# tensorflow/recommenders

Hardware: NVIDIA H100
Metric: queries/sec brute-force top-K (1Mx64 candidates) (higher is better)
Workload: dtype f32 (fp16 wgmma screening, fp32 accumulate + exact fp32 re-scoring)

## Files before the change

### recommenders_b200/csrc/common.cuh

```cuda
#pragma once
#include <cuda_runtime.h>
#include <stdint.h>
#include <stdio.h>
#include <stdarg.h>

#include "../../include/tfrs_b200.h"

namespace tfrs {

void set_error(const char* fmt, ...);
void count_launch(int n = 1);

#define TFRS_CHECK_ARG(cond, ...)                          \
  do {                                                     \
    if (!(cond)) {                                         \
      ::tfrs::set_error(__VA_ARGS__);                      \
      return TFRS_ERR_INVALID_ARG;                         \
    }                                                      \
  } while (0)

#define TFRS_CUDA(expr)                                                                          \
  do {                                                                                           \
    cudaError_t e__ = (expr);                                                                    \
    if (e__ != cudaSuccess) {                                                                    \
      ::tfrs::set_error("%s:%d %s -> %s", __FILE__, __LINE__, #expr, cudaGetErrorString(e__));   \
      return TFRS_ERR_CUDA;                                                                      \
    }                                                                                            \
  } while (0)

#define TFRS_LAUNCH_CHECK()                                                                      \
  do {                                                                                           \
    ::tfrs::count_launch();                                                                      \
    cudaError_t e__ = cudaGetLastError();                                                        \
    if (e__ != cudaSuccess) {                                                                    \
      ::tfrs::set_error("%s:%d kernel launch -> %s", __FILE__, __LINE__, cudaGetErrorString(e__)); \
      return TFRS_ERR_CUDA;                                                                      \
    }                                                                                            \
  } while (0)

static inline size_t align_up(size_t x, size_t a) { return (x + a - 1) / a * a; }
static inline int64_t ceil_div(int64_t a, int64_t b) { return (a + b - 1) / b; }

__host__ __device__ __forceinline__ bool better(float sa, long long ia, float sb, long long ib) {
  return (sa > sb) || (sa == sb && ia < ib);
}

__device__ __forceinline__ float finite_abs(float v) {
  const float a = fabsf(v);
  return a < INFINITY ? a : 0.f;
}

int sm_count();

static inline unsigned elementwise_grid(long long n) {
  const long long want = ceil_div(n, 256), cap = (long long)sm_count() * 16;
  return (unsigned)(want < cap ? want : cap);
}

int reduce_parts(const float* partial, long long M, long long N, int parts, float* out, long long ld, cudaStream_t st);
int reduce_loss(const float* v, long long n, long long stride, float* loss, cudaStream_t st);

typedef int (*ThrHook)(void* ctx, float* thr, const float* margin, const float* cut, const int* qexp, const int* exp_corpus,
                       long long Q, cudaStream_t st);
int tc_topk_sharded_local(const float* q, int64_t Q, const float* corpus, const void* index_buf, int64_t N, int d, int k,
                          int64_t index_offset, float* out_scores, int64_t* out_idx, void* ws, size_t ws_bytes, void* stream,
                          ThrHook hook, void* hook_ctx);

struct DeviceOnce {
  unsigned char done_[64] = {};
  int dev_ = 0;
  bool need() { if (cudaGetDevice(&dev_) != cudaSuccess) dev_ = 0; dev_ &= 63; return __atomic_load_n(&done_[dev_], __ATOMIC_ACQUIRE) == 0; }
  void done() { __atomic_store_n(&done_[dev_], (unsigned char)1, __ATOMIC_RELEASE); }
};
#define TFRS_DYN_SMEM(kernel, bytes)                                                                              \
  do {                                                                                                            \
    static ::tfrs::DeviceOnce once__;                                                                             \
    if (once__.need()) {                                                                                          \
      TFRS_CUDA(cudaFuncSetAttribute(kernel, cudaFuncAttributeMaxDynamicSharedMemorySize, (int)(bytes)));         \
                                \
      TFRS_CUDA(cudaFuncSetAttribute(kernel, cudaFuncAttributePreferredSharedMemoryCarveout,                        \
                                     (int)cudaSharedmemCarveoutMaxShared));                                         \
      once__.done();                                                                                              \
    }                                                                                                             \
  } while (0)

}
```

### recommenders_b200/csrc/rowselect.cuh

```cuda
#pragma once
#include "common.cuh"
#include <limits.h>

namespace tfrs {

constexpr int RS_THREADS = 256;

__device__ __forceinline__ void bitonic_sort_desc(float* bs, long long* bi, int P) {
  for (int size = 2; size <= P; size <<= 1) {
    for (int stride = size >> 1; stride > 0; stride >>= 1) {
      for (int t = threadIdx.x; t < (P >> 1); t += blockDim.x) {
        int lo = 2 * t - (t & (stride - 1));
        int hi = lo + stride;
        bool desc = ((lo & size) == 0);
        float sl = bs[lo], sh = bs[hi];
        long long il = bi[lo], ih = bi[hi];
        bool hi_better = better(sh, ih, sl, il);
        bool lo_better = better(sl, il, sh, ih);
        if (desc ? hi_better : lo_better) { bs[lo] = sh; bs[hi] = sl; bi[lo] = ih; bi[hi] = il; }
      }
      __syncthreads();
    }
  }
}

static inline int pow2_ceil(int x) { int p = 1; while (p < x) p <<= 1; return p; }
static inline int rowselect_cap(int k) { int c = pow2_ceil(2 * k); return c < 1024 ? 1024 : c; }
static inline size_t rowselect_smem(int cap, size_t extra) { return (size_t)cap * 12 + extra; }

template <class Provider>
__global__ void __launch_bounds__(RS_THREADS)
row_topk_kernel(Provider prov, int k, int cap, float* __restrict__ out_s, long long* __restrict__ out_i,
                int out_ld) {
  extern __shared__ __align__(16) unsigned char rs_smem[];
  long long* bi = reinterpret_cast<long long*>(rs_smem);
  float* bs = reinterpret_cast<float*>(rs_smem + (size_t)cap * 8);
  void* extra = rs_smem + (size_t)cap * 12;
  __shared__ int cnt_sh;
  __shared__ float thr_s_sh;
  __shared__ long long thr_i_sh;
  __shared__ int full_sh;

  const int row = blockIdx.x;
  const int tid = threadIdx.x;
  if (tid == 0) { cnt_sh = 0; full_sh = 0; thr_s_sh = 0.f; thr_i_sh = 0; }
  prov.begin(row, extra);
  __syncthreads();

  const long long total = prov.count(row);
  const int min_room = cap / 4;
  long long pos = 0;
  while (pos < total) {
    __syncthreads();
    const int cnt0 = cnt_sh;
    const bool full = full_sh != 0;
    const float ts = thr_s_sh;
    const long long ti = thr_i_sh;
    __syncthreads();
    const int slab = (int)min((long long)(cap - cnt0), total - pos);
    for (int t = tid; t < slab; t += RS_THREADS) {
      float s; long long i;
      prov.get(row, pos + t, s, i);
      if (!full || better(s, i, ts, ti)) {
        int p = atomicAdd(&cnt_sh, 1);
        bs[p] = s; bi[p] = i;
      }
    }
    __syncthreads();
    pos += slab;
    const int cnt = cnt_sh;
    if (pos < total && cap - cnt >= min_room) continue;
    int P = 2; while (P < cnt) P <<= 1;
    for (int t = cnt + tid; t < P; t += RS_THREADS) { bs[t] = -INFINITY; bi[t] = LLONG_MAX; }
    __syncthreads();
    if (cnt > 1) bitonic_sort_desc(bs, bi, P);
    if (tid == 0) {
      int keep = cnt < k ? cnt : k;
      cnt_sh = keep;
      if (keep == k) { full_sh = 1; thr_s_sh = bs[k - 1]; thr_i_sh = bi[k - 1]; }
    }
  }
  __syncthreads();
  const int n_out = cnt_sh;
  for (int t = tid; t < n_out; t += RS_THREADS) {
    out_s[(long long)row * out_ld + t] = bs[t];
    out_i[(long long)row * out_ld + t] = bi[t];
  }
}

}
```

### recommenders_b200/csrc/topk_tc.cu

```cuda
#include <cuda_fp16.h>
#include <math.h>
#include <stdlib.h>
#include <type_traits>
#include "rowselect.cuh"
#include "tc_ptx.cuh"

namespace tfrs {
namespace tc {

constexpr int TILE_N = 128;
constexpr int TILE_M = 128;
constexpr int QBLK = 256;
constexpr int KSLAB = 64;
constexpr int SLAB_BYTES = TILE_N * 128;
constexpr int HEADER_BYTES = 1024;
constexpr int THREADS = 512;
constexpr int CONSUMER_WARPS = 16;
constexpr int CAND_CAP = 2048;
constexpr int MAX_SAMPLE_STRIDE = 4;
constexpr int FIN_MAX_PARTS = 2 * 132;
constexpr int MAX_BINS = 1024;
constexpr int FP16_TARGET = 15;
constexpr float E_REL = 0.00108f;
constexpr float E_ACC = 0.00013f;

struct SideStats {
  unsigned int max_norm2_bits;
  unsigned int amax_bits;
  int exp;
  int pad;
};
enum { SAMPLE_STRIDED = 0, SAMPLE_NORM = 1 };
constexpr long long NORM_SAMPLE_MIN_N = 1ll << 19;
constexpr int NORM_SAMPLE_DIV = 8;
constexpr double NORM_SAMPLE_TAIL = 1e-4;
constexpr double NORM_SAMPLE_MIN_PHI = 0.35;
constexpr int NORM_PROBES = 256, NORM_PROBE_K = 100;
constexpr float NORM_PROBE_MIN_MEAN = 0.35f, NORM_PROBE_MIN_EACH = 0.25f;
struct IndexHeader {
  SideStats st;
  int d, d_pad, kb, sample;
  long long n, n_tiles;
  float phi;
  float probe_mean, probe_min;
};
__host__ __device__ inline long long norm_sample_tiles(long long N) {
  return N >= NORM_SAMPLE_MIN_N && N < (1ll << 31) ? N / NORM_SAMPLE_DIV / 128 : 0;
}

__device__ __forceinline__ int rescale_exp(float amax) {
  int x = 0;
  if (!(amax > 0.f) || !(amax < INFINITY)) return 0;
  (void)frexpf(amax, &x);
  return FP16_TARGET - x;
}

// ... 529 lines not shown
    int c = 0;
#pragma unroll
    for (int j = 0; j < KPL; ++j) c += (key[j] >= cand) ? 1 : 0;
    c = __reduce_add_sync(0xffffffffu, c);
    if (c >= k) prefix = cand;
  }
  return prefix;
}
__device__ __forceinline__ unsigned int warp_kth_largest_smem(const unsigned int* keys, int n, int k, int lane, unsigned int prefix, int top_bit) {
  for (int bit = top_bit; bit >= 0; --bit) {
    const unsigned int cand = prefix | (1u << bit);
    int c = 0;
    for (int t = lane; t < n; t += 32) c += (keys[t] >= cand) ? 1 : 0;
    c = __reduce_add_sync(0xffffffffu, c);
    if (c >= k) prefix = cand;
  }
  return prefix;
}

template <int KPL>
__device__ __forceinline__ void thresholds_of_row(const float* __restrict__ binmax, int bins_ld, int n_bins, int k, int k_filter,
                                                  const float* __restrict__ margin, float* __restrict__ thr, float* __restrict__ thr_safe,
                                                  unsigned int* __restrict__ overflow, unsigned int* __restrict__ retry, long long row, int lane) {
  const float* src = binmax + row * bins_ld;
  unsigned int key[KPL];
#pragma unroll
  for (int j = 0; j < KPL; ++j) { const int i = j * 32 + lane; key[j] = i < n_bins ? f2key(__ldg(src + i)) : 0u; }
  const float safe = key2f(warp_kth_largest_regs<KPL>(key, k)) - margin[row];
  const float filter = k_filter < k ? key2f(warp_kth_largest_regs<KPL>(key, k_filter)) - margin[row] : safe;
  if (lane == 0) { thr[row] = filter; thr_safe[row] = safe; overflow[row] = 0; retry[row] = 0; }
}
template <int KPL>
__global__ void __launch_bounds__(256)
tc_threshold_kernel(const float* __restrict__ binmax, int bins_ld, int n_bins, int k, int k_filter, const float* __restrict__ margin,
                    float* __restrict__ thr, float* __restrict__ thr_safe, unsigned int* __restrict__ overflow,
                    unsigned int* __restrict__ retry, long long Q, const IndexHeader* __restrict__ hdr, int n_bins_norm) {
  const int lane = threadIdx.x & 31;
  const long long row = ((long long)blockIdx.x * 256 + threadIdx.x) >> 5;
  if (row >= Q) return;
  if (n_bins_norm > 0 && hdr->sample == SAMPLE_NORM) { n_bins = n_bins_norm; k_filter = k; }
  if (KPL > 16 && n_bins <= 512) thresholds_of_row<16>(binmax, bins_ld, n_bins, k, k_filter, margin, thr, thr_safe, overflow, retry, row, lane);
  else thresholds_of_row<KPL>(binmax, bins_ld, n_bins, k, k_filter, margin, thr, thr_safe, overflow, retry, row, lane);
}

enum { FIN_TOPK = 0, FIN_EXCLUDE = 1, FIN_COUNT = 2 };
constexpr int FW_WARPS = 4;

struct FinParams {
  const float* q; const float* corpus; int d; int k; long long index_offset; long long N; long long Q;
  const unsigned int* count; const float* cand_s; const unsigned int* cand_i; int segs; int cap_part;
  const float* cut; float* thr; const float* thr_safe; unsigned int* overflow;
  unsigned int* retry; int retry_pass;
  int cap_keys, cap_band;
  unsigned int* band_idx; int* band_n;
  int allow_short;
  float* out_s; long long* out_i;
  const long long* identifiers; const long long* exclusions; int n_excl; int k_out;
  const float* pos; const int* qexp; const IndexHeader* hdr; int* out_count;
};

__device__ __forceinline__ float exact_score(const float* __restrict__ qs, const float* __restrict__ c, int d) {
  float acc = 0.f;
  if ((d & 31) == 0) {
    for (int kk = 0; kk < d; kk += 32) {
      float4 cv[8];
#pragma unroll
      for (int u = 0; u < 8; ++u) cv[u] = __ldg(reinterpret_cast<const float4*>(c + kk) + u);
#pragma unroll
      for (int u = 0; u < 8; ++u) {
        acc = fmaf(qs[kk + 4 * u], cv[u].x, acc); acc = fmaf(qs[kk + 4 * u + 1], cv[u].y, acc);
        acc = fmaf(qs[kk + 4 * u + 2], cv[u].z, acc); acc = fmaf(qs[kk + 4 * u + 3], cv[u].w, acc);
      }
    }
  } else if ((d & 3) == 0) {
    for (int kk = 0; kk < d; kk += 4) {
      const float4 cv = __ldg(reinterpret_cast<const float4*>(c + kk));
      acc = fmaf(qs[kk], cv.x, acc); acc = fmaf(qs[kk + 1], cv.y, acc);
      acc = fmaf(qs[kk + 2], cv.z, acc); acc = fmaf(qs[kk + 3], cv.w, acc);
    }
  } else {
    for (int kk = 0; kk < d; ++kk) acc = fmaf(qs[kk], __ldg(c + kk), acc);
  }
  return acc;
}

__device__ __forceinline__ void exact_score2(const float* __restrict__ qs, const float* __restrict__ c0, const float* __restrict__ c1,
                                             int d, float& s0, float& s1) {
  if ((d & 31) == 0) {
    float a0 = 0.f, a1 = 0.f;
    for (int kk = 0; kk < d; kk += 32) {
      float4 u0[8], u1[8];
#pragma unroll
      for (int u = 0; u < 8; ++u) { u0[u] = __ldg(reinterpret_cast<const float4*>(c0 + kk) + u); u1[u] = __ldg(reinterpret_cast<const float4*>(c1 + kk) + u); }
#pragma unroll
      for (int u = 0; u < 8; ++u) {
        const float q0 = qs[kk + 4 * u], q1 = qs[kk + 4 * u + 1], q2 = qs[kk + 4 * u + 2], q3 = qs[kk + 4 * u + 3];
        a0 = fmaf(q0, u0[u].x, a0); a1 = fmaf(q0, u1[u].x, a1);
        a0 = fmaf(q1, u0[u].y, a0); a1 = fmaf(q1, u1[u].y, a1);
        a0 = fmaf(q2, u0[u].z, a0); a1 = fmaf(q2, u1[u].z, a1);
        a0 = fmaf(q3, u0[u].w, a0); a1 = fmaf(q3, u1[u].w, a1);
      }
    }
    s0 = a0; s1 = a1;
  } else {
    s0 = exact_score(qs, c0, d); s1 = exact_score(qs, c1, d);
  }
}

__device__ __forceinline__ void exclude_rerank(const unsigned long long* srt, int kf, unsigned long long* akey, long long row,
                                               const FinParams& p, int lane) {
  for (int t = lane; t < kf; t += 32) {
    const unsigned long long e = srt[t];
    const float s = key2f((unsigned int)(e >> 32));
    const long long gi = (long long)rank_key_index(e) + p.index_offset;
    const long long ident = p.identifiers ? __ldg(p.identifiers + gi) : gi;
    bool isin = false;
    for (int x = 0; x < p.n_excl; ++x) isin |= (__ldg(p.exclusions + row * p.n_excl + x) == ident);
    const float adj = (isin ? s - 1.0e5f : s) + 0.0f;
    akey[t] = ((unsigned long long)f2key(adj) << 32) | (unsigned long long)(0xFFFFFFFFu - (unsigned int)t);
  }
  __syncwarp();
  for (int t = lane; t < kf; t += 32) {
    const unsigned long long mine = akey[t];
    int rank = 0;
    for (int j = 0; j < kf; ++j) rank += (akey[j] > mine) ? 1 : 0;
    if (rank < p.k_out) {
      const unsigned long long e = srt[t];
      p.out_s[row * p.k_out + rank] = rank_key_score(e);
      p.out_i[row * p.k_out + rank] = (long long)rank_key_index(e) + p.index_offset;
    }
  }
}

__host__ __device__ inline size_t sel_warp_bytes(int cap_keys, int segs) {
  return (size_t)cap_keys * 4 + (size_t)cap_keys * 2 + (size_t)((segs + 1 + 3) & ~3) * 4;
}
constexpr int SEL_WARPS = 8;

__device__ __forceinline__ bool load_record(const FinParams& p, long long row, const int* soff, int rec, int total_rec,
                                            unsigned int& ix0, float (&sc)[8]) {
  if (rec >= total_rec) return false;
  int lo = 0, hi = p.segs;
  while (hi - lo > 1) { const int mid = (lo + hi) >> 1; if (soff[mid] <= rec) lo = mid; else hi = mid; }
  const long long at = (row * p.segs + lo) * p.cap_part + (rec - soff[lo]);
  ix0 = __ldg(p.cand_i + at);
  const float4 s0 = __ldg(reinterpret_cast<const float4*>(p.cand_s + at * 8));
  const float4 s1 = __ldg(reinterpret_cast<const float4*>(p.cand_s + at * 8) + 1);
  sc[0] = s0.x; sc[1] = s0.y; sc[2] = s0.z; sc[3] = s0.w; sc[4] = s1.x; sc[5] = s1.y; sc[6] = s1.z; sc[7] = s1.w;
  return true;
}

template <int MODE>
__global__ void __launch_bounds__(SEL_WARPS * 32)
tc_select_kernel(const FinParams p) {
  extern __shared__ __align__(16) unsigned char fsm[];
  const int warp = threadIdx.x >> 5, lane = threadIdx.x & 31;
  const long long row = (long long)blockIdx.x * SEL_WARPS + warp;
  if (row >= p.Q || (p.retry_pass && p.retry[row] == 0u)) return;
  unsigned char* base = fsm + (size_t)warp * sel_warp_bytes(p.cap_keys, p.segs);
  unsigned int* keys = reinterpret_cast<unsigned int*>(base);
  unsigned short* loc = reinterpret_cast<unsigned short*>(keys + p.cap_keys);
  int* soff = reinterpret_cast<int*>(loc + p.cap_keys);
  const unsigned int n32 = (unsigned int)p.N;
  unsigned int* band = p.band_idx + row * p.cap_band;

  int carry = 0; bool bad = false;
  for (int s0 = 0; s0 < p.segs; s0 += 32) {
    const int s = s0 + lane;
    int c = 0;
    if (s < p.segs) {
      const unsigned int cc = __ldg(p.count + row * p.segs + s);
      if (cc > (unsigned int)p.cap_part) bad = true; else c = (int)cc;
    }
    const int inc = warp_incl_scan(c, lane);
    if (s < p.segs) soff[s + 1] = carry + inc;
    carry += __shfl_sync(0xffffffffu, inc, 31);
  }
  if (lane == 0) soff[0] = 0;
  if (__any_sync(0xffffffffu, bad)) {
    if (lane == 0) { p.overflow[row] = 1; p.band_n[row] = 0; }
    return;
  }
  __syncwarp();
  const int total_rec = soff[p.segs];
  const float thr_row = p.thr[row];
  if (MODE != FIN_COUNT && total_rec >= 8192) {
    if (lane == 0) { p.overflow[row] = 1; p.band_n[row] = 0; }
    return;
  }

  if (MODE == FIN_COUNT) {
    const float eps = 0.5f * p.cut[row];
    const float pos_s = ldexpf(p.pos[row], p.hdr->st.exp + p.qexp[row]);
    const float hi = pos_s + eps, lo_b = pos_s - eps;
    int definite = 0, m = 0;
    for (int rb = 0; rb < total_rec; rb += 32) {
      unsigned int ix0 = 0, amb = 0; int cnt = 0; float sc[8];
      if (load_record(p, row, soff, rb + lane, total_rec, ix0, sc)) {
#pragma unroll
        for (int j = 0; j < 8; ++j) {
          const bool real = ix0 + j < n32;
          definite += (real && sc[j] > hi) ? 1 : 0;
          const bool a = real && sc[j] > lo_b && !(sc[j] > hi);
          amb |= a ? (1u << j) : 0u; cnt += a ? 1 : 0;
        }
      }
      const int incl = warp_incl_scan(cnt, lane);
      const int tot = __shfl_sync(0xffffffffu, incl, 31);
      if (m + tot <= p.cap_band) {
        int at_pos = m + incl - cnt;
#pragma unroll
        for (int j = 0; j < 8; ++j)
          if (amb & (1u << j)) { band[at_pos] = ix0 + j; ++at_pos; }
      }
      m += tot;
    }
    definite = __reduce_add_sync(0xffffffffu, definite);
    if (lane == 0) {
      if (definite >= p.k) { p.out_count[row] = p.k; p.band_n[row] = 0; p.overflow[row] = 0; }
      else if (m > p.cap_band) { p.overflow[row] = 1; p.band_n[row] = 0; }
      else { p.out_count[row] = definite; p.band_n[row] = m; p.overflow[row] = 0; }
    }
    return;
  }

  int n = 0;
  unsigned int kmax = 0u, kmin = 0xFFFFFFFFu;
  for (int rb = 0; rb < total_rec; rb += 32) {
    float sc[8]; unsigned int ix0 = 0, keep = 0; int cnt = 0;
    if (load_record(p, row, soff, rb + lane, total_rec, ix0, sc)) {
#pragma unroll
      for (int j = 0; j < 8; ++j) {
        const bool kp = sc[j] >= thr_row && ix0 + j < n32;
        keep |= kp ? (1u << j) : 0u; cnt += kp ? 1 : 0;
      }
    }
    const int incl = warp_incl_scan(cnt, lane);
    const int tot = __shfl_sync(0xffffffffu, incl, 31);
    if (n + tot <= p.cap_keys) {
      int at_pos = n + incl - cnt;
#pragma unroll
      for (int j = 0; j < 8; ++j) {
        if (keep & (1u << j)) {
          const unsigned int key = f2key(sc[j] + 0.0f);
          kmax = max(kmax, key); kmin = min(kmin, key);
          keys[at_pos] = key;
          loc[at_pos] = (unsigned short)(((rb + lane) << 3) | j);
          ++at_pos;
        }
      }
    }
    n += tot;
  }
  auto miss = [&]() {
    if (lane == 0) {
      const float safe = p.thr_safe[row];
      if (thr_row > safe) { p.retry[row] = 1; p.thr[row] = safe; } else p.overflow[row] = 1;
      p.band_n[row] = 0;
    }
  };
  if (n > p.cap_keys) { if (lane == 0) { p.overflow[row] = 1; p.band_n[row] = 0; } return; }
  if (n < p.k && !p.allow_short) { miss(); return; }
  __syncwarp();
  if (n < p.k) {
    const bool fits = n <= p.cap_band;
    for (int t = lane; t < n && fits; t += 32) {
      const unsigned int l = loc[t];
      const int rec = (int)(l >> 3);
      int lo = 0, hi = p.segs;
      while (hi - lo > 1) { const int mid = (lo + hi) >> 1; if (soff[mid] <= rec) lo = mid; else hi = mid; }
      band[t] = __ldg(p.cand_i + (row * p.segs + lo) * p.cap_part + (rec - soff[lo])) + (l & 7u);
    }
    if (lane == 0) { p.overflow[row] = fits ? 0u : 1u; p.band_n[row] = fits ? n : 0; }
    return;
  }
  kmax = __reduce_max_sync(0xffffffffu, kmax); kmin = __reduce_min_sync(0xffffffffu, kmin);
  unsigned int tau_key;
  {
    const unsigned int diff = kmax ^ kmin;
    const int top = diff ? (31 - __clz(diff)) : -1;
    const unsigned int prefix0 = top >= 31 ? 0u : (top < 0 ? kmax : (kmax & ~((2u << top) - 1u)));
    if (n <= 512) {
      unsigned int kr[16];
#pragma unroll
      for (int j = 0; j < 16; ++j) { const int t = j * 32 + lane; kr[j] = t < n ? keys[t] : 0u; }
      tau_key = warp_kth_largest_regs<16>(kr, p.k, prefix0, top);
    } else if (n <= 1024) {
      unsigned int kr[32];
#pragma unroll
      for (int j = 0; j < 32; ++j) { const int t = j * 32 + lane; kr[j] = t < n ? keys[t] : 0u; }
      tau_key = warp_kth_largest_regs<32>(kr, p.k, prefix0, top);
    } else {
      tau_key = warp_kth_largest_smem(keys, n, p.k, lane, prefix0, top);
    }
  }
  const float lim = key2f(tau_key) - p.cut[row];
  if (!p.allow_short && (!(lim >= thr_row) || !(lim > -INFINITY))) { miss(); return; }
  const unsigned int lim_key = f2key(lim + 0.0f);
  const unsigned int lt_mask = (1u << lane) - 1u;
  int m = 0;
  for (int tb = 0; tb < n; tb += 32) {
    const int t = tb + lane;
    const bool kp = t < n && keys[t] >= lim_key;
    const unsigned int vote = __ballot_sync(0xffffffffu, kp);
    if (kp) {
      const int at_pos = m + __popc(vote & lt_mask);
      if (at_pos < p.cap_band) {
        const unsigned int l = loc[t];
        const int rec = (int)(l >> 3);
        int lo = 0, hi = p.segs;
        while (hi - lo > 1) { const int mid = (lo + hi) >> 1; if (soff[mid] <= rec) lo = mid; else hi = mid; }
        band[at_pos] = __ldg(p.cand_i + (row * p.segs + lo) * p.cap_part + (rec - soff[lo])) + (l & 7u);
      }
    }
    m += __popc(vote);
  }
  if (lane == 0) {
    if (m > p.cap_band) { p.overflow[row] = 1; p.band_n[row] = 0; }
    else { p.overflow[row] = 0; p.band_n[row] = m; }
  }
}

constexpr int RS_BLOCK = 128;
template <int MODE>
__global__ void __launch_bounds__(RS_BLOCK)
tc_rescore_kernel(const FinParams p) {
  extern __shared__ __align__(16) unsigned char rsm[];
  unsigned long long* sk = reinterpret_cast<unsigned long long*>(rsm);
  float* qs = reinterpret_cast<float*>(sk + p.cap_band);
  unsigned long long* srt = reinterpret_cast<unsigned long long*>(qs + ((p.d + 3) & ~3));
  __shared__ int greater_sh;
  const long long row = blockIdx.x;
  const int tid = threadIdx.x;
  if (p.overflow[row] != 0) return;
  const int m = p.band_n[row];
  if (MODE == FIN_COUNT && m == 0) return;
  for (int t = tid; t < p.d; t += RS_BLOCK) qs[t] = p.q[row * p.d + t];
  if (tid == 0) greater_sh = 0;
  __syncthreads();
  const unsigned int* band = p.band_idx + row * p.cap_band;
  if (MODE == FIN_COUNT) {
    const float pos = p.pos[row];
    int g = 0;
    for (int t = tid; t < m; t += RS_BLOCK) g += (exact_score(qs, p.corpus + (long long)band[t] * p.d, p.d) > pos) ? 1 : 0;
    g = __reduce_add_sync(0xffffffffu, g);
    if ((tid & 31) == 0 && g) atomicAdd(&greater_sh, g);
    __syncthreads();
    if (tid == 0) { const int c = p.out_count[row] + greater_sh; p.out_count[row] = c < p.k ? c : p.k; }
    return;
  }
  if (p.d == 64) {
    constexpr int RPB = RS_BLOCK / 8;
    constexpr int MAXR = 8;
    const int sub = tid & 7, grp = tid >> 3;
    for (int t0 = 0; t0 < m; t0 += RPB * MAXR) {
      float4 a[MAXR], b[MAXR];
#pragma unroll
      for (int r = 0; r < MAXR; ++r) {
        const int t = t0 + r * RPB + grp;
        if (t < m) {
          const float4* src = reinterpret_cast<const float4*>(p.corpus + (long long)band[t] * 64) + sub * 2;
          a[r] = __ldg(src); b[r] = __ldg(src + 1);
        }
      }
      const float q0 = qs[sub * 8], q1 = qs[sub * 8 + 1], q2 = qs[sub * 8 + 2], q3 = qs[sub * 8 + 3];
      const float q4 = qs[sub * 8 + 4], q5 = qs[sub * 8 + 5], q6 = qs[sub * 8 + 6], q7 = qs[sub * 8 + 7];
#pragma unroll
      for (int r = 0; r < MAXR; ++r) {
        const int t = t0 + r * RPB + grp;
        const bool live = t < m;
        float acc = 0.f;
#pragma unroll
        for (int step = 0; step < 8; ++step) {
          if (sub == step && live) {
            acc = fmaf(q0, a[r].x, acc); acc = fmaf(q1, a[r].y, acc); acc = fmaf(q2, a[r].z, acc); acc = fmaf(q3, a[r].w, acc);
            acc = fmaf(q4, b[r].x, acc); acc = fmaf(q5, b[r].y, acc); acc = fmaf(q6, b[r].z, acc); acc = fmaf(q7, b[r].w, acc);
          }
          acc = __shfl_sync(0xffffffffu, acc, (threadIdx.x & 24) | step);
        }
        if (live && sub == 0) sk[t] = rank_key(acc, band[t]);
      }
    }
  } else {
    for (int t = tid; t < m; t += RS_BLOCK) {
      const unsigned int idx = band[t];
      sk[t] = rank_key(exact_score(qs, p.corpus + (long long)idx * p.d, p.d), idx);
    }
  }
  __syncthreads();
  if (MODE == FIN_TOPK && m < p.k)
    for (int t = m + tid; t < p.k; t += RS_BLOCK) { p.out_s[row * p.k + t] = -INFINITY; p.out_i[row * p.k + t] = LLONG_MAX; }
  for (int t = tid; t < m; t += RS_BLOCK) {
    const unsigned long long mine = sk[t];
    int rank = 0;
#pragma unroll 4
    for (int j = 0; j < m; ++j) rank += (sk[j] > mine) ? 1 : 0;
    if (rank < p.k) {
      if (MODE == FIN_TOPK) {
        p.out_s[row * p.k + rank] = rank_key_score(mine);
        p.out_i[row * p.k + rank] = (long long)rank_key_index(mine) + p.index_offset;
      } else {
        srt[rank] = mine;
      }
    }
  }
  if (MODE == FIN_EXCLUDE) {
    __syncthreads();
    if (tid < 32) exclude_rerank(srt, p.k, srt + p.k, row, p, tid);
  }
}

__global__ void __launch_bounds__(FW_WARPS * 32)
tc_exclude_fallback_kernel(const FinParams p, const float* __restrict__ tmp_s, const long long* __restrict__ tmp_i,
                           const unsigned int* __restrict__ was_fallback) {
  extern __shared__ __align__(16) unsigned char fsm[];
  const int warp = threadIdx.x >> 5, lane = threadIdx.x & 31;
  const long long row = (long long)blockIdx.x * FW_WARPS + warp;
  if (row >= p.Q || was_fallback[row] == 0) return;
  unsigned long long* srt = reinterpret_cast<unsigned long long*>(fsm) + (size_t)warp * 2 * p.k;
  unsigned long long* akey = srt + p.k;
  for (int t = lane; t < p.k; t += 32)
    srt[t] = rank_key(tmp_s[row * p.k + t], (unsigned int)(tmp_i[row * p.k + t] - p.index_offset));
  __syncwarp();
  exclude_rerank(srt, p.k, akey, row, p, lane);
}

struct FallbackProvider {
  const float* q; const float* corpus; long long N; int d; long long index_offset; const unsigned int* overflow;
  float* qs;
  __device__ void begin(int row, void* extra) {
    qs = reinterpret_cast<float*>(extra);
    if (overflow[row] != 0) for (int t = threadIdx.x; t < d; t += blockDim.x) qs[t] = q[(long long)row * d + t];
  }
  __device__ long long count(int row) const { return overflow[row] != 0 ? N : 0; }
  __device__ void get(int, long long t, float& s, long long& i) const {
    const float* c = corpus + t * d;
    float acc = 0.f;
    for (int kk = 0; kk < d; ++kk) acc = fmaf(qs[kk], __ldg(c + kk), acc);
    s = acc; i = index_offset + t;
  }
};

__global__ void __launch_bounds__(256)
tc_count_fallback_kernel(const float* __restrict__ q, const float* __restrict__ corpus, long long N, int d, int k,
                         const float* __restrict__ pos, const unsigned int* __restrict__ overflow, int* __restrict__ out_count) {
  __shared__ float qs[128];
  __shared__ int total;
  const int row = blockIdx.x;
  if (overflow[row] == 0) return;
  for (int t = threadIdx.x; t < d; t += 256) qs[t] = q[(long long)row * d + t];
  if (threadIdx.x == 0) total = 0;
  __syncthreads();
  const float ps = pos[row];
  int c = 0;
  for (long long t = threadIdx.x; t < N; t += 256) {
    const float* cr = corpus + t * d;
    float acc = 0.f;
    for (int kk = 0; kk < d; ++kk) acc = fmaf(qs[kk], __ldg(cr + kk), acc);
    c += (acc + 0.0f > ps) ? 1 : 0;
  }
  c = __reduce_add_sync(0xffffffffu, c);
// ... 88 lines not shown
  }
  {
    const double lambda = (double)k * pl.stride / (pl.parts_full * 2.0);
    const double want = 2.0 * lambda + 12.0 * sqrt(lambda) + 8.0;
    int p2 = 32; while (p2 < want && p2 < 512) p2 <<= 1;
    pl.cap_part = p2;
    int ck = 1024; while (ck < 1.6 * 1.3 * k * pl.stride && ck < 4096) ck <<= 1;
    pl.cap_keys = ck;
    pl.cap_band = ck / 2;
  }
  pl.smem = (size_t)(2 + pl.stages) * pl.kb * SLAB_BYTES + 1024  + 256 ;
  size_t o = 0;
  auto take = [&](size_t bytes) { size_t r = o; o += align_up(bytes, 1024); return r; };
  pl.o_qimg = take((size_t)pl.nqb * 2 * pl.kb * SLAB_BYTES);
  pl.o_margin = take((size_t)pl.Qp * 4);
  pl.o_cut = take((size_t)pl.Qp * 4);
  pl.o_thr = take((size_t)pl.Qp * 4);
  pl.o_qexp = take((size_t)pl.Qp * 4);
  pl.o_count = take((size_t)pl.Qp * pl.parts_full * 2 * 4);
  pl.o_ovf = take((size_t)pl.Qp * 4);
  pl.o_binmax = take((size_t)pl.Qp * pl.bins_ld * 4);
  pl.o_cand = take((size_t)pl.Qp * pl.parts_full * 2 * pl.cap_part * (8 * 4 + 4));
  pl.o_tmp = take((size_t)Q * k * 12);
  pl.o_band = take((size_t)pl.Qp * pl.cap_band * 4);
  pl.o_bandn = take((size_t)pl.Qp * 4);
  pl.o_thr_safe = take((size_t)pl.Qp * 4);
  pl.o_retry = take((size_t)pl.Qp * 4);
  pl.total = o;
  return true;
}

template <int KB, int STAGES>
static int launch_scans(const Plan& pl, ScanParams sp, cudaStream_t st, int mode) {
  auto ks = tc_scan_kernel<KB, STAGES, MODE_SAMPLE>;
  auto kf = tc_scan_kernel<KB, STAGES, MODE_FILTER>;
  TFRS_DYN_SMEM(ks, (int)pl.smem);
  TFRS_DYN_SMEM(kf, (int)pl.smem);
  if (mode == MODE_SAMPLE) {
    sp.parts = pl.parts_sample; sp.n_seq = pl.n_sample; sp.stride = pl.stride;
    ks<<<(unsigned)(pl.nqb * sp.parts), THREADS, pl.smem, st>>>(sp);
  } else {
    sp.parts = pl.parts_full; sp.n_seq = (int)pl.n_tiles; sp.stride = 1;
    kf<<<(unsigned)(pl.nqb * sp.parts), THREADS, pl.smem, st>>>(sp);
  }
  TFRS_LAUNCH_CHECK();
  return TFRS_OK;
}

static int launch_scan_mode(const Plan& pl, const ScanParams& sp, cudaStream_t st, int mode) {
  if (pl.kb == 1) return launch_scans<1, 6>(pl, sp, st, mode);
  return launch_scans<2, 4>(pl, sp, st, mode);
}

template <int MODE>
static int launch_finalize(FinParams fp, const Plan& pl, ScanParams sp, bool retry, cudaStream_t st) {
  auto ksel = tc_select_kernel<MODE>;
  auto krs = tc_rescore_kernel<MODE>;
  TFRS_DYN_SMEM(ksel, (int)(SEL_WARPS * sel_warp_bytes(4096, FIN_MAX_PARTS)));
  ksel<<<(unsigned)ceil_div(fp.Q, SEL_WARPS), SEL_WARPS * 32, SEL_WARPS * sel_warp_bytes(fp.cap_keys, fp.segs), st>>>(fp);
  TFRS_LAUNCH_CHECK();
  if (retry) {
    sp.retry = fp.retry;
    const int rc = launch_scan_mode(pl, sp, st, MODE_FILTER);
    if (rc) return rc;
    fp.retry_pass = 1;
    ksel<<<(unsigned)ceil_div(fp.Q, SEL_WARPS), SEL_WARPS * 32, SEL_WARPS * sel_warp_bytes(fp.cap_keys, fp.segs), st>>>(fp);
    TFRS_LAUNCH_CHECK();
  }
  const size_t rs_smem = (size_t)fp.cap_band * 8 + (size_t)((fp.d + 3) & ~3) * 4 + (MODE == FIN_EXCLUDE ? (size_t)fp.k * 16 : 0);
  TFRS_DYN_SMEM(krs, 64 * 1024);
  krs<<<(unsigned)fp.Q, RS_BLOCK, rs_smem, st>>>(fp);
  TFRS_LAUNCH_CHECK();
  return TFRS_OK;
}

struct Call {
  int mode;
  const float* q; long long Q; const float* corpus; const void* index_buf; long long N; int d; int k; long long index_offset;
  void* ws; size_t ws_bytes; cudaStream_t st;
  float* out_s; long long* out_i;
  const long long* identifiers; const long long* exclusions; int n_excl; int k_out;
  const float* pos; int* out_count;
  ThrHook hook; void* hook_ctx; int allow_short;
};

static int run_call(const Call& c) {
  Plan pl;
  if (!make_plan(c.Q, c.N, c.d, c.k, pl)) {
    set_error("topk_tc: shape (Q=%lld N=%lld d=%d k=%d) is outside the tensor-core path; use tfrs_topk_scan_f32",
              c.Q, c.N, c.d, c.k);
    return TFRS_ERR_UNSUPPORTED;
  }
  if (!c.ws || c.ws_bytes < pl.total + 16) { set_error("topk_tc: workspace too small (%zu < %zu)", c.ws_bytes, pl.total + 16); return TFRS_ERR_WORKSPACE_TOO_SMALL; }
  TFRS_CHECK_ARG((c.d & 3) != 0 || (reinterpret_cast<uintptr_t>(c.corpus) & 15) == 0,
                 "topk_tc: the corpus must be 16-byte aligned when d %% 4 == 0 (d=%d); pass an aligned copy", c.d);
  cudaStream_t st = c.st;
  unsigned char* w = (unsigned char*)(((uintptr_t)c.ws + 15) & ~(uintptr_t)15);
  unsigned char* qimg = w + pl.o_qimg;
  float* margin = (float*)(w + pl.o_margin);
  float* cut = (float*)(w + pl.o_cut);
  float* thr = (float*)(w + pl.o_thr);
  int* qexp = (int*)(w + pl.o_qexp);
  unsigned int* count = (unsigned int*)(w + pl.o_count);
  unsigned int* ovf = (unsigned int*)(w + pl.o_ovf);
  float* binmax = (float*)(w + pl.o_binmax);
  float* cand_s = (float*)(w + pl.o_cand);
  unsigned int* cand_i = (unsigned int*)(w + pl.o_cand + (size_t)pl.Qp * pl.parts_full * 2 * pl.cap_part * 32);
  float* tmp_s = (float*)(w + pl.o_tmp);
  long long* tmp_i = (long long*)(w + pl.o_tmp + align_up((size_t)c.Q * c.k * 4, 8));
  float* thr_safe = (float*)(w + pl.o_thr_safe);
  unsigned int* retry = (unsigned int*)(w + pl.o_retry);
  const IndexHeader* hdr = (const IndexHeader*)c.index_buf;
  const unsigned char* cimg = (const unsigned char*)c.index_buf + HEADER_BYTES;
  const int k_filter = (c.mode == FIN_COUNT || c.hook) ? c.k : pl.k_filter;

  prof_mark(st, 0);
  tc_qprep_kernel<<<(unsigned)ceil_div(pl.Qp * 32, 256), 256, 0, st>>>(c.q, c.Q, pl.Qp, c.d, pl.kb, hdr, qimg, margin, cut, qexp);
  TFRS_LAUNCH_CHECK();
  ScanParams sp{};
  sp.qimg = qimg; sp.cimg = cimg; sp.Q = c.Q; sp.N = c.N; sp.nqb = pl.nqb; sp.n_tiles = pl.n_tiles;
  sp.binmax = binmax; sp.bins_ld = pl.bins_ld; sp.group = pl.group; sp.bins_per_part = pl.bins_per_part;
  sp.hdr = hdr;
  sp.simg = pl.n_bins_norm > 0 ? cimg + pl.n_tiles * pl.kb * (long long)SLAB_BYTES : nullptr;
  sp.n_seq_norm = pl.n_seq_norm; sp.group_norm = pl.group_norm; sp.bins_per_part_norm = pl.bins_per_part_norm;
  sp.thr = thr; sp.count = count; sp.cand_s = cand_s; sp.cand_i = cand_i; sp.cap_part = pl.cap_part;
  prof_mark(st, 1);
  int rc = launch_scan_mode(pl, sp, st, MODE_SAMPLE);
  if (rc) return rc;
  if (pl.n_bins <= 512 && pl.n_bins_norm <= 512)
    tc_threshold_kernel<16><<<(unsigned)ceil_div(c.Q * 32, 256), 256, 0, st>>>(binmax, pl.bins_ld, pl.n_bins, c.k, k_filter, margin,
                                                                                 thr, thr_safe, ovf, retry, c.Q, hdr, pl.n_bins_norm);
  else
    tc_threshold_kernel<32><<<(unsigned)ceil_div(c.Q * 32, 256), 256, 0, st>>>(binmax, pl.bins_ld, pl.n_bins, c.k, k_filter, margin,
                                                                                 thr, thr_safe, ovf, retry, c.Q, hdr, pl.n_bins_norm);
  TFRS_LAUNCH_CHECK();
  if (c.hook) {
    rc = c.hook(c.hook_ctx, thr, margin, cut, qexp, &hdr->st.exp, c.Q, st);
    if (rc) return rc;
  }
  prof_mark(st, 2);
  rc = launch_scan_mode(pl, sp, st, MODE_FILTER);
  if (rc) return rc;
  prof_mark(st, 3);
  if (FILTER_ABLATION != FILTER_FULL) { prof_mark(st, 4); return TFRS_OK; }
  FinParams fp{};
  fp.q = c.q; fp.corpus = c.corpus; fp.d = c.d; fp.k = c.k; fp.index_offset = c.index_offset; fp.N = c.N; fp.Q = c.Q;
  fp.count = count; fp.cand_s = cand_s; fp.cand_i = cand_i; fp.segs = pl.parts_full * 2; fp.cap_part = pl.cap_part;
  fp.cut = cut; fp.thr = thr; fp.thr_safe = thr_safe; fp.overflow = ovf; fp.retry = retry; fp.out_s = c.out_s; fp.out_i = c.out_i;
  fp.cap_keys = pl.cap_keys; fp.cap_band = pl.cap_band; fp.allow_short = c.allow_short;
  fp.band_idx = (unsigned int*)(w + pl.o_band); fp.band_n = (int*)(w + pl.o_bandn);
  fp.identifiers = c.identifiers; fp.exclusions = c.exclusions; fp.n_excl = c.n_excl; fp.k_out = c.k_out;
  fp.pos = c.pos; fp.qexp = qexp; fp.hdr = hdr; fp.out_count = c.out_count;
  const bool may_retry = k_filter < c.k;
  if (c.mode == FIN_TOPK) rc = launch_finalize<FIN_TOPK>(fp, pl, sp, may_retry, st);
  else if (c.mode == FIN_EXCLUDE) rc = launch_finalize<FIN_EXCLUDE>(fp, pl, sp, may_retry, st);
  else rc = launch_finalize<FIN_COUNT>(fp, pl, sp, false, st);
  if (rc) return rc;
  if (c.mode == FIN_COUNT) {
    tc_count_fallback_kernel<<<(unsigned)c.Q, 256, 0, st>>>(c.q, c.corpus, c.N, c.d, c.k, c.pos, ovf, c.out_count);
    TFRS_LAUNCH_CHECK();
  } else {
    FallbackProvider prov{c.q, c.corpus, c.N, c.d, c.index_offset, ovf, nullptr};
    int cap = rowselect_cap(c.k);
    TFRS_DYN_SMEM(row_topk_kernel<FallbackProvider>, 64 * 1024);
    float* fs = c.mode == FIN_TOPK ? c.out_s : tmp_s;
    long long* fi = c.mode == FIN_TOPK ? c.out_i : tmp_i;
    row_topk_kernel<FallbackProvider><<<(unsigned)c.Q, RS_THREADS, rowselect_smem(cap, (size_t)c.d * 4), st>>>(prov, c.k, cap, fs, fi, c.k);
    TFRS_LAUNCH_CHECK();
    if (c.mode == FIN_EXCLUDE) {
      tc_exclude_fallback_kernel<<<(unsigned)ceil_div(c.Q, FW_WARPS), FW_WARPS * 32, (size_t)FW_WARPS * 2 * c.k * 8, st>>>(fp, tmp_s, tmp_i, ovf);
      TFRS_LAUNCH_CHECK();
    }
  }
  prof_mark(st, 4);
  return TFRS_OK;
}

}
}

using namespace tfrs;
using namespace tfrs::tc;

extern "C" size_t tfrs_index_bytes(int64_t N, int d) {
  if (N <= 0 || d <= 0 || d > 128) return 0;
  int kb = (d + KSLAB - 1) / KSLAB;
  return (size_t)HEADER_BYTES + (size_t)(ceil_div(N, TILE_N) + norm_sample_tiles(N)) * kb * SLAB_BYTES;
}

extern "C" int tfrs_index_build(const float* corpus, int64_t N, int d, void* index_buf, size_t index_bytes, void* stream) {
  TFRS_CHECK_ARG(corpus && index_buf && N > 0 && d > 0, "index_build: bad arguments");
  if (d > 128) { set_error("index_build: d=%d > 128 is not supported by the tensor-core path", d); return TFRS_ERR_UNSUPPORTED; }
  TFRS_CHECK_ARG(index_bytes >= tfrs_index_bytes(N, d), "index_build: buffer too small");
  TFRS_CHECK_ARG((reinterpret_cast<uintptr_t>(index_buf) & 15) == 0, "index_build: buffer must be 16-byte aligned");
  cudaStream_t st = (cudaStream_t)stream;
  IndexHeader h{};
  h.d = d; h.kb = (d + KSLAB - 1) / KSLAB; h.d_pad = h.kb * KSLAB; h.n = N; h.n_tiles = ceil_div(N, TILE_N);
  TFRS_CUDA(cudaMemsetAsync(index_buf, 0, HEADER_BYTES, st));
  header_kernel<<<1, 1, 0, st>>>(reinterpret_cast<IndexHeader*>(index_buf), h);
  TFRS_LAUNCH_CHECK();
  SideStats* cst = &reinterpret_cast<IndexHeader*>(index_buf)->st;
  const unsigned sgrid = (unsigned)(sm_count() * 8);
  corpus_stats_kernel<0><<<sgrid, 256, 0, st>>>(corpus, N, d, cst);
  TFRS_LAUNCH_CHECK();
  side_exp_kernel<<<1, 1, 0, st>>>(cst);
  TFRS_LAUNCH_CHECK();
  const long long s_tiles = norm_sample_tiles(N);
  if (s_tiles == 0) {
    corpus_stats_kernel<1><<<sgrid, 256, 0, st>>>(corpus, N, d, cst);
    TFRS_LAUNCH_CHECK();
  }
  auto image = [&](long long rows, long long tiles, unsigned char* dst, const int* rowmap) {
    const long long chunks = tiles * TILE_N * (long long)h.kb * 8;
    const unsigned blocks = (unsigned)(ceil_div(chunks, 256) < (1 << 20) ? ceil_div(chunks, 256) : (1 << 20));
    tile_image_kernel<<<blocks, 256, 0, st>>>(corpus, rows, d, h.kb, tiles, cst, dst, rowmap);
  };
  unsigned char* img = (unsigned char*)index_buf + HEADER_BYTES;
  image(N, h.n_tiles, img, nullptr);
  TFRS_LAUNCH_CHECK();
  if (s_tiles == 0) return TFRS_OK;
// ... 175 lines not shown
```

Measured before the change: 3.274 million.

## Add PDL launches, prefetch select loads, and team-based multi-row rescore kernel

Adds programmatic dependent launch (griddepcontrol) to the select, rescore and fallback row-topk kernels so each kernel's prologue can overlap the tail of the previous one. Software-prefetches the next record in the select kernel's band and filter loops, and batches four ballot rounds in band compaction. Restructures the rescore kernel so a block of four warps serves one to four query rows depending on Q, with named barriers, shuffle-distributed band indices and multi-key ranking. This aims to cut launch gaps and latency stalls in the finalize stage, at the cost of more register pressure and more complex barrier logic.

```diff
diff --git a/recommenders_b200/csrc/common.cuh b/recommenders_b200/csrc/common.cuh
--- a/recommenders_b200/csrc/common.cuh
+++ b/recommenders_b200/csrc/common.cuh
@@ -40,6 +40,17 @@
 
 static inline size_t align_up(size_t x, size_t a) { return (x + a - 1) / a * a; }
 static inline int64_t ceil_div(int64_t a, int64_t b) { return (a + b - 1) / b; }
+
+__device__ __forceinline__ void grid_dependency_wait() {
+#if defined(__CUDA_ARCH__) && __CUDA_ARCH__ >= 900
+  asm volatile("griddepcontrol.wait;" ::: "memory");
+#endif
+}
+__device__ __forceinline__ void grid_dependents_launch() {
+#if defined(__CUDA_ARCH__) && __CUDA_ARCH__ >= 900
+  asm volatile("griddepcontrol.launch_dependents;" :::);
+#endif
+}
 
 __host__ __device__ __forceinline__ bool better(float sa, long long ia, float sb, long long ib) {
   return (sa > sb) || (sa == sb && ia < ib);
diff --git a/recommenders_b200/csrc/rowselect.cuh b/recommenders_b200/csrc/rowselect.cuh
--- a/recommenders_b200/csrc/rowselect.cuh
+++ b/recommenders_b200/csrc/rowselect.cuh
@@ -43,6 +43,7 @@
 
   const int row = blockIdx.x;
   const int tid = threadIdx.x;
+  grid_dependency_wait();
   if (tid == 0) { cnt_sh = 0; full_sh = 0; thr_s_sh = 0.f; thr_i_sh = 0; }
   prov.begin(row, extra);
   __syncthreads();
diff --git a/recommenders_b200/csrc/topk_tc.cu b/recommenders_b200/csrc/topk_tc.cu
--- a/recommenders_b200/csrc/topk_tc.cu
+++ b/recommenders_b200/csrc/topk_tc.cu
@@ -2,6 +2,7 @@
 #include <math.h>
 #include <stdlib.h>
 #include <type_traits>
+#include <utility>
 #include "rowselect.cuh"
 #include "tc_ptx.cuh"
 
@@ -637,6 +638,7 @@
   const float* cut; float* thr; const float* thr_safe; unsigned int* overflow;
   unsigned int* retry; int retry_pass;
   int cap_keys, cap_band;
+  int rs_team;
   unsigned int* band_idx; int* band_n;
   int allow_short;
   float* out_s; long long* out_i;
@@ -739,6 +741,8 @@
 __global__ void __launch_bounds__(SEL_WARPS * 32)
 tc_select_kernel(const FinParams p) {
   extern __shared__ __align__(16) unsigned char fsm[];
+  grid_dependency_wait();
+  grid_dependents_launch();
   const int warp = threadIdx.x >> 5, lane = threadIdx.x & 31;
   const long long row = (long long)blockIdx.x * SEL_WARPS + warp;
   if (row >= p.Q || (p.retry_pass && p.retry[row] == 0u)) return;
@@ -779,9 +783,12 @@
     const float pos_s = ldexpf(p.pos[row], p.hdr->st.exp + p.qexp[row]);
     const float hi = pos_s + eps, lo_b = pos_s - eps;
     int definite = 0, m = 0;
+    unsigned int ix0 = 0; float sc[8];
+    bool have = load_record(p, row, soff, lane, total_rec, ix0, sc);
     for (int rb = 0; rb < total_rec; rb += 32) {
-      unsigned int ix0 = 0, amb = 0; int cnt = 0; float sc[8];
-      if (load_record(p, row, soff, rb + lane, total_rec, ix0, sc)) {
+      unsigned int nix0 = 0, amb = 0; int cnt = 0; float nsc[8];
+      const bool nhave = load_record(p, row, soff, rb + 32 + lane, total_rec, nix0, nsc);
+      if (have) {
 #pragma unroll
         for (int j = 0; j < 8; ++j) {
           const bool real = ix0 + j < n32;
@@ -799,6 +806,9 @@
           if (amb & (1u << j)) { band[at_pos] = ix0 + j; ++at_pos; }
       }
       m += tot;
+      have = nhave; ix0 = nix0;
+#pragma unroll
+      for (int j = 0; j < 8; ++j) sc[j] = nsc[j];
     }
     definite = __reduce_add_sync(0xffffffffu, definite);
     if (lane == 0) {
@@ -811,9 +821,12 @@
 
   int n = 0;
   unsigned int kmax = 0u, kmin = 0xFFFFFFFFu;
+  float sc[8]; unsigned int ix0 = 0;
+  bool have = load_record(p, row, soff, lane, total_rec, ix0, sc);
   for (int rb = 0; rb < total_rec; rb += 32) {
-    float sc[8]; unsigned int ix0 = 0, keep = 0; int cnt = 0;
-    if (load_record(p, row, soff, rb + lane, total_rec, ix0, sc)) {
+    float nsc[8]; unsigned int nix0 = 0, keep = 0; int cnt = 0;
+    const bool nhave = load_record(p, row, soff, rb + 32 + lane, total_rec, nix0, nsc);
+    if (have) {
 #pragma unroll
       for (int j = 0; j < 8; ++j) {
         const bool kp = sc[j] >= thr_row && ix0 + j < n32;
@@ -836,6 +849,9 @@
       }
     }
     n += tot;
+    have = nhave; ix0 = nix0;
+#pragma unroll
+    for (int j = 0; j < 8; ++j) sc[j] = nsc[j];
   }
   auto miss = [&]() {
     if (lane == 0) {
@@ -884,21 +900,26 @@
   const unsigned int lim_key = f2key(lim + 0.0f);
   const unsigned int lt_mask = (1u << lane) - 1u;
   int m = 0;
-  for (int tb = 0; tb < n; tb += 32) {
-    const int t = tb + lane;
-    const bool kp = t < n && keys[t] >= lim_key;
-    const unsigned int vote = __ballot_sync(0xffffffffu, kp);
-    if (kp) {
-      const int at_pos = m + __popc(vote & lt_mask);
-      if (at_pos < p.cap_band) {
+  for (int tb0 = 0; tb0 < n; tb0 += 128) {
+    int at[4]; unsigned int v[4];
+#pragma unroll
+    for (int u = 0; u < 4; ++u) {
+      const int t = tb0 + u * 32 + lane;
+      const bool kp = t < n && keys[t] >= lim_key;
+      const unsigned int vote = __ballot_sync(0xffffffffu, kp);
+      at[u] = kp ? m + __popc(vote & lt_mask) : p.cap_band;
+      if (at[u] < p.cap_band) {
         const unsigned int l = loc[t];
         const int rec = (int)(l >> 3);
         int lo = 0, hi = p.segs;
         while (hi - lo > 1) { const int mid = (lo + hi) >> 1; if (soff[mid] <= rec) lo = mid; else hi = mid; }
-        band[at_pos] = __ldg(p.cand_i + (row * p.segs + lo) * p.cap_part + (rec - soff[lo])) + (l & 7u);
+        v[u] = __ldg(p.cand_i + (row * p.segs + lo) * p.cap_part + (rec - soff[lo])) + (l & 7u);
       }
-    }
-    m += __popc(vote);
+      m += __popc(vote);
+    }
+#pragma unroll
+    for (int u = 0; u < 4; ++u)
+      if (at[u] < p.cap_band) band[at[u]] = v[u];
   }
   if (lane == 0) {
     if (m > p.cap_band) { p.overflow[row] = 1; p.band_n[row] = 0; }
@@ -906,92 +927,136 @@
   }
 }
 
-constexpr int RS_BLOCK = 128;
+constexpr int RS_WARPS = 4;
+constexpr int RS_MIN_BLOCKS = 8;
+__host__ __device__ inline size_t rs_team_bytes(int cap_band, int d, int k, int mode) {
+  return (size_t)cap_band * 8 + (size_t)((d + 3) & ~3) * 4 + (mode == FIN_EXCLUDE ? (size_t)k * 16 : 0) + 16;
+}
+static int rs_team(long long Q, int d) {
+  if (d != 64) return RS_WARPS;
+  const long long slots = (long long)RS_MIN_BLOCKS * RS_WARPS * sm_count();
+  return Q * 4 <= slots ? 4 : (Q * 2 <= slots ? 2 : 1);
+}
+template <int MODE, int KEYS>
+__device__ __forceinline__ void rank_band(const FinParams& p, const unsigned long long* sk, int m, int tt, int nt, long long row,
+                                          unsigned long long* srt) {
+  for (int t0 = tt; t0 < m; t0 += KEYS * nt) {
+    unsigned long long mine[KEYS]; int rank[KEYS];
+#pragma unroll
+    for (int u = 0; u < KEYS; ++u) { const int t = t0 + u * nt; mine[u] = t < m ? sk[t] : ~0ull; rank[u] = 0; }
+#pragma unroll 4
+    for (int j = 0; j < m; ++j) {
+      const unsigned long long e = sk[j];
+#pragma unroll
+      for (int u = 0; u < KEYS; ++u) rank[u] += (e > mine[u]) ? 1 : 0;
+    }
+#pragma unroll
+    for (int u = 0; u < KEYS; ++u) {
+      if (t0 + u * nt < m && rank[u] < p.k) {
+        if (MODE == FIN_TOPK) {
+          p.out_s[row * p.k + rank[u]] = rank_key_score(mine[u]);
+          p.out_i[row * p.k + rank[u]] = (long long)rank_key_index(mine[u]) + p.index_offset;
+        } else {
+          srt[rank[u]] = mine[u];
+        }
+      }
+    }
+  }
+}
 template <int MODE>
-__global__ void __launch_bounds__(RS_BLOCK)
+__global__ void __launch_bounds__(RS_WARPS * 32, RS_MIN_BLOCKS)
 tc_rescore_kernel(const FinParams p) {
   extern __shared__ __align__(16) unsigned char rsm[];
-  unsigned long long* sk = reinterpret_cast<unsigned long long*>(rsm);
+  grid_dependency_wait();
+  grid_dependents_launch();
+  const int tw = p.rs_team;
+  const int warp = threadIdx.x >> 5, lane = threadIdx.x & 31;
+  const int team = warp / tw, tw_warp = warp % tw, tt = tw_warp * 32 + lane, nt = tw * 32;
+  static_assert(RS_WARPS == 4, "team_sync names the barriers of two 2-warp teams");
+  const long long row = (long long)blockIdx.x * (RS_WARPS / tw) + team;
+  if (row >= p.Q) return;
+  unsigned long long* sk = reinterpret_cast<unsigned long long*>(rsm + (size_t)team * rs_team_bytes(p.cap_band, p.d, p.k, MODE));
   float* qs = reinterpret_cast<float*>(sk + p.cap_band);
   unsigned long long* srt = reinterpret_cast<unsigned long long*>(qs + ((p.d + 3) & ~3));
-  __shared__ int greater_sh;
-  const long long row = blockIdx.x;
-  const int tid = threadIdx.x;
-  if (p.overflow[row] != 0) return;
+  int* part = reinterpret_cast<int*>(MODE == FIN_EXCLUDE ? reinterpret_cast<unsigned char*>(srt + 2 * p.k)
+                                                         : reinterpret_cast<unsigned char*>(srt));
+  auto team_sync = [&]() {
+    if (tw == 1) __syncwarp();
+    else if (tw == RS_WARPS) __syncthreads();
+    else if (team == 0) asm volatile("bar.sync 1, 64;" ::: "memory");
+    else asm volatile("bar.sync 2, 64;" ::: "memory");
+  };
+  const unsigned int* band = p.band_idx + row * p.cap_band;
+  const unsigned int ovf = p.overflow[row];
   const int m = p.band_n[row];
+  const int sub = lane & 7, grp = lane >> 3;
+  unsigned int bi = band[tw_warp * 8 + sub];
+  for (int t = tt; t < p.d; t += nt) qs[t] = p.q[row * p.d + t];
+  if (ovf != 0) return;
   if (MODE == FIN_COUNT && m == 0) return;
-  for (int t = tid; t < p.d; t += RS_BLOCK) qs[t] = p.q[row * p.d + t];
-  if (tid == 0) greater_sh = 0;
-  __syncthreads();
-  const unsigned int* band = p.band_idx + row * p.cap_band;
+  team_sync();
   if (MODE == FIN_COUNT) {
     const float pos = p.pos[row];
     int g = 0;
-    for (int t = tid; t < m; t += RS_BLOCK) g += (exact_score(qs, p.corpus + (long long)band[t] * p.d, p.d) > pos) ? 1 : 0;
+    for (int t = tt; t < m; t += nt) g += (exact_score(qs, p.corpus + (long long)band[t] * p.d, p.d) > pos) ? 1 : 0;
     g = __reduce_add_sync(0xffffffffu, g);
-    if ((tid & 31) == 0 && g) atomicAdd(&greater_sh, g);
-    __syncthreads();
-    if (tid == 0) { const int c = p.out_count[row] + greater_sh; p.out_count[row] = c < p.k ? c : p.k; }
+    if (lane == 0) part[tw_warp] = g;
+    team_sync();
+    if (tt == 0) {
+      int c = p.out_count[row];
+      for (int w = 0; w < tw; ++w) c += part[w];
+      p.out_count[row] = c < p.k ? c : p.k;
+    }
     return;
   }
   if (p.d == 64) {
-    constexpr int RPB = RS_BLOCK / 8;
-    constexpr int MAXR = 8;
-    const int sub = tid & 7, grp = tid >> 3;
-    for (int t0 = 0; t0 < m; t0 += RPB * MAXR) {
-      float4 a[MAXR], b[MAXR];
-#pragma unroll
-      for (int r = 0; r < MAXR; ++r) {
-        const int t = t0 + r * RPB + grp;
+    constexpr int ROUNDS = 2;
+    const float4* qv = reinterpret_cast<const float4*>(qs) + sub * 2;
+    for (int t0 = tw_warp * 8; t0 < m; t0 += 8 * tw) {
+      float4 a[ROUNDS], b[ROUNDS];
+#pragma unroll
+      for (int r = 0; r < ROUNDS; ++r) {
+        const int t = t0 + r * 4 + grp;
+        const unsigned int ix = __shfl_sync(0xffffffffu, bi, r * 4 + grp);
         if (t < m) {
-          const float4* src = reinterpret_cast<const float4*>(p.corpus + (long long)band[t] * 64) + sub * 2;
+          const float4* src = reinterpret_cast<const float4*>(p.corpus + (long long)ix * 64) + sub * 2;
           a[r] = __ldg(src); b[r] = __ldg(src + 1);
         }
       }
-      const float q0 = qs[sub * 8], q1 = qs[sub * 8 + 1], q2 = qs[sub * 8 + 2], q3 = qs[sub * 8 + 3];
-      const float q4 = qs[sub * 8 + 4], q5 = qs[sub * 8 + 5], q6 = qs[sub * 8 + 6], q7 = qs[sub * 8 + 7];
-#pragma unroll
-      for (int r = 0; r < MAXR; ++r) {
-        const int t = t0 + r * RPB + grp;
+      const unsigned int bi_cur = bi;
+      if (t0 + 8 * tw < m) bi = band[t0 + 8 * tw + sub];
+#pragma unroll
+      for (int r = 0; r < ROUNDS; ++r) {
+        const int t = t0 + r * 4 + grp;
         const bool live = t < m;
         float acc = 0.f;
 #pragma unroll
         for (int step = 0; step < 8; ++step) {
           if (sub == step && live) {
-            acc = fmaf(q0, a[r].x, acc); acc = fmaf(q1, a[r].y, acc); acc = fmaf(q2, a[r].z, acc); acc = fmaf(q3, a[r].w, acc);
-            acc = fmaf(q4, b[r].x, acc); acc = fmaf(q5, b[r].y, acc); acc = fmaf(q6, b[r].z, acc); acc = fmaf(q7, b[r].w, acc);
+            const float4 qa = qv[0], qb = qv[1];
+            acc = fmaf(qa.x, a[r].x, acc); acc = fmaf(qa.y, a[r].y, acc); acc = fmaf(qa.z, a[r].z, acc); acc = fmaf(qa.w, a[r].w, acc);
+            acc = fmaf(qb.x, b[r].x, acc); acc = fmaf(qb.y, b[r].y, acc); acc = fmaf(qb.z, b[r].z, acc); acc = fmaf(qb.w, b[r].w, acc);
           }
-          acc = __shfl_sync(0xffffffffu, acc, (threadIdx.x & 24) | step);
+          acc = __shfl_sync(0xffffffffu, acc, (lane & 24) | step);
         }
-        if (live && sub == 0) sk[t] = rank_key(acc, band[t]);
+        const unsigned int ix = __shfl_sync(0xffffffffu, bi_cur, r * 4 + grp);
+        if (live && sub == 0) sk[t] = rank_key(acc, ix);
       }
     }
   } else {
-    for (int t = tid; t < m; t += RS_BLOCK) {
+    for (int t = tt; t < m; t += nt) {
       const unsigned int idx = band[t];
       sk[t] = rank_key(exact_score(qs, p.corpus + (long long)idx * p.d, p.d), idx);
     }
   }
-  __syncthreads();
+  team_sync();
   if (MODE == FIN_TOPK && m < p.k)
-    for (int t = m + tid; t < p.k; t += RS_BLOCK) { p.out_s[row * p.k + t] = -INFINITY; p.out_i[row * p.k + t] = LLONG_MAX; }
-  for (int t = tid; t < m; t += RS_BLOCK) {
-    const unsigned long long mine = sk[t];
-    int rank = 0;
-#pragma unroll 4
-    for (int j = 0; j < m; ++j) rank += (sk[j] > mine) ? 1 : 0;
-    if (rank < p.k) {
-      if (MODE == FIN_TOPK) {
-        p.out_s[row * p.k + rank] = rank_key_score(mine);
-        p.out_i[row * p.k + rank] = (long long)rank_key_index(mine) + p.index_offset;
-      } else {
-        srt[rank] = mine;
-      }
-    }
-  }
+    for (int t = m + tt; t < p.k; t += nt) { p.out_s[row * p.k + t] = -INFINITY; p.out_i[row * p.k + t] = LLONG_MAX; }
+  if (MODE != FIN_EXCLUDE && tw == 1) rank_band<MODE, 4>(p, sk, m, tt, nt, row, srt);
+  else rank_band<MODE, 1>(p, sk, m, tt, nt, row, srt);
   if (MODE == FIN_EXCLUDE) {
-    __syncthreads();
-    if (tid < 32) exclude_rerank(srt, p.k, srt + p.k, row, p, tid);
+    team_sync();
+    if (tw_warp == 0) exclude_rerank(srt, p.k, srt + p.k, row, p, lane);
   }
 }
 
@@ -1186,24 +1251,39 @@
   return launch_scans<2, 4>(pl, sp, st, mode);
 }
 
+template <typename... Params, typename... Args>
+static cudaError_t launch_dependent(void (*kernel)(Params...), dim3 grid, dim3 block, size_t smem, cudaStream_t st, Args&&... args) {
+  cudaLaunchAttribute attr[1];
+  attr[0].id = cudaLaunchAttributeProgrammaticStreamSerialization;
+  attr[0].val.programmaticStreamSerializationAllowed = 1;
+  cudaLaunchConfig_t cfg = {};
+  cfg.gridDim = grid; cfg.blockDim = block; cfg.dynamicSmemBytes = smem; cfg.stream = st;
+  cfg.attrs = attr; cfg.numAttrs = 1;
+  return cudaLaunchKernelEx(&cfg, kernel, std::forward<Args>(args)...);
+}
+
 template <int MODE>
 static int launch_finalize(FinParams fp, const Plan& pl, ScanParams sp, bool retry, cudaStream_t st) {
   auto ksel = tc_select_kernel<MODE>;
   auto krs = tc_rescore_kernel<MODE>;
   TFRS_DYN_SMEM(ksel, (int)(SEL_WARPS * sel_warp_bytes(4096, FIN_MAX_PARTS)));
-  ksel<<<(unsigned)ceil_div(fp.Q, SEL_WARPS), SEL_WARPS * 32, SEL_WARPS * sel_warp_bytes(fp.cap_keys, fp.segs), st>>>(fp);
+  const dim3 sel_grid((unsigned)ceil_div(fp.Q, SEL_WARPS)), sel_block(SEL_WARPS * 32);
+  const size_t sel_smem = SEL_WARPS * sel_warp_bytes(fp.cap_keys, fp.segs);
+  TFRS_CUDA(launch_dependent(ksel, sel_grid, sel_block, sel_smem, st, fp));
   TFRS_LAUNCH_CHECK();
   if (retry) {
     sp.retry = fp.retry;
     const int rc = launch_scan_mode(pl, sp, st, MODE_FILTER);
     if (rc) return rc;
     fp.retry_pass = 1;
-    ksel<<<(unsigned)ceil_div(fp.Q, SEL_WARPS), SEL_WARPS * 32, SEL_WARPS * sel_warp_bytes(fp.cap_keys, fp.segs), st>>>(fp);
+    TFRS_CUDA(launch_dependent(ksel, sel_grid, sel_block, sel_smem, st, fp));
     TFRS_LAUNCH_CHECK();
   }
-  const size_t rs_smem = (size_t)fp.cap_band * 8 + (size_t)((fp.d + 3) & ~3) * 4 + (MODE == FIN_EXCLUDE ? (size_t)fp.k * 16 : 0);
-  TFRS_DYN_SMEM(krs, 64 * 1024);
-  krs<<<(unsigned)fp.Q, RS_BLOCK, rs_smem, st>>>(fp);
+  TFRS_DYN_SMEM(krs, (int)(RS_WARPS * rs_team_bytes(2048, 128, 256, MODE)));
+  fp.rs_team = rs_team(fp.Q, fp.d);
+  const int per_cta = RS_WARPS / fp.rs_team;
+  TFRS_CUDA(launch_dependent(krs, dim3((unsigned)ceil_div(fp.Q, per_cta)), dim3(RS_WARPS * 32),
+                             per_cta * rs_team_bytes(fp.cap_band, fp.d, fp.k, MODE), st, fp));
   TFRS_LAUNCH_CHECK();
   return TFRS_OK;
 }
@@ -1299,7 +1379,8 @@
     TFRS_DYN_SMEM(row_topk_kernel<FallbackProvider>, 64 * 1024);
     float* fs = c.mode == FIN_TOPK ? c.out_s : tmp_s;
     long long* fi = c.mode == FIN_TOPK ? c.out_i : tmp_i;
-    row_topk_kernel<FallbackProvider><<<(unsigned)c.Q, RS_THREADS, rowselect_smem(cap, (size_t)c.d * 4), st>>>(prov, c.k, cap, fs, fi, c.k);
+    TFRS_CUDA(launch_dependent(row_topk_kernel<FallbackProvider>, dim3((unsigned)c.Q), dim3(RS_THREADS),
+                               rowselect_smem(cap, (size_t)c.d * 4), st, prov, c.k, cap, fs, fi, c.k));
     TFRS_LAUNCH_CHECK();
     if (c.mode == FIN_EXCLUDE) {
       tc_exclude_fallback_kernel<<<(unsigned)ceil_div(c.Q, FW_WARPS), FW_WARPS * 32, (size_t)FW_WARPS * 2 * c.k * 8, st>>>(fp, tmp_s, tmp_i, ovf);
```

New measurement: 3.364 million, median of 6. +2.7%, better.
